# a-rtemis99/hpc_suffix_array

Hardware: AMD Instinct MI355X
Metric: suffixes sorted/sec + ms/doubling-round, 1 GiB input at 1/2/4/8 MI355X (higher is better)
Workload: dtype u32

## Files before the change

hpc_suffix_array_amd/_native.py:

```python
from __future__ import annotations

import ctypes
import os
import subprocess

PKG_DIR = os.path.dirname(os.path.abspath(__file__))
LIB_PATH = os.path.join(PKG_DIR, "lib", "libsa_hip.so")
LIB_PATH = os.environ.get("SA_LIB_PATH", LIB_PATH)
CSRC = os.path.join(PKG_DIR, "csrc")

SA_MAX_ROUNDS = 64
KERNEL_KINDS = ["init", "hist_first", "hist_keys", "scan", "scatter_first", "scatter_keys",
                "heads", "heads_scan", "rerank", "seg_count", "seg_scan", "seg_write", "alphabet", "pack",
                "sort_u", "windows", "local_sort", "pivot_keys", "pivot_count", "pivot_write"]
SCHEDULE_PACKED = 0
SCHEDULE_REFERENCE = 1
ROUND1_AUTO = 0
ROUND1_LSD = 1
ROUND1_BUCKETED = 2
SA_K_COUNT = len(KERNEL_KINDS)
FIND_AUTO = 0
FIND_LANE = 1
FIND_WAVE = 2
FIND_LANE_MAX = 3584
# ... 101 lines not shown
            "round_ms": list(self.round_ms[:r]),
            "distinct": [int(x) for x in self.distinct[:r]],
            "passes": list(self.passes[:r]),
            "sorted_n": [int(x) for x in self.sorted_n[:r]],
            "prefix_len": [int(x) for x in self.prefix_len[:r]],
            "schedule": "reference" if self.schedule == SCHEDULE_REFERENCE else "packed",
            "init_chars": self.init_chars,
            "sigma": self.sigma,
            "sparse_ranks": bool(self.sparse_ranks),
            "round1": {ROUND1_LSD: "lsd", ROUND1_BUCKETED: "bucketed", 3: "pivot"}.get(self.round1, "lsd"),
            "largest_window": self.largest_window,
            "round1_segments": {0: "exact", 1: "padded", 2: "padded-overflow", 3: "striped-records",
                                4: "striped-records-overflow"}.get(self.round1_segments, "exact"),
            "round1_layout": {"compact": bool(self.round1_layout & 1), "pk8": bool(self.round1_layout & 2),
                              "xq": bool(self.round1_layout & 4), "eonly": bool(self.round1_layout & 8)},
            "reference_model_bytes": int(self.model_bytes),
            "round_bytes": [int(x) for x in self.round_bytes[:r]],
            "round1_windows": [int(x) for x in self.round1_windows],
            "alphabet": {0: "exact", 1: "sampled", 2: "refuted"}.get(self.alphabet, "exact"),
            "kernels": {k: {"ms": self.kern_ms[i], "launches": int(self.kern_launches[i]),
                            "bytes": int(self.kern_bytes[i])} for i, k in enumerate(KERNEL_KINDS)},
        }


DIST_OK = 0
DIST_UNSUPPORTED = 1
DIST_UNBALANCED = 2


class SaDistInfo(ctypes.Structure):
# ... 182 lines not shown
```

hpc_suffix_array_amd/csrc/sa_build.hip:

```cpp
#include <hip/hip_runtime.h>

#include <algorithm>
#include <atomic>
#include <chrono>
#include <cstdarg>
#include <cstdio>
#include <cstdlib>
#include <cstring>
#include <mutex>
#include <string>
#include <thread>
#include <vector>

#include "../../include/sa_hip.h"

#ifndef SA_ALPHA_GRID
#define SA_ALPHA_GRID 2048
#endif

#include "sa_bucket.h"
#include "sa_check.h"
#include "sa_kernels.h"
#include "sa_lcp.h"
#include "sa_limits.h"
// ... 122 lines not shown
    uint32_t* counts = nullptr;
    uint32_t* words = nullptr;
    uint32_t* alpha = nullptr;
    uint16_t* code = nullptr;
    uint32_t* host_words = nullptr;
    hipEvent_t ev[sa::kEvPool + sa::kRoundEv + 1];
    int ev_ready = 0;
    sa::DistState* dist = nullptr;
    uint32_t dbg = 0;
    int32_t span_extra = 0;
    int32_t tune = 0;
    bool dna = false;
    bool alpha_prove = false;
    bool alpha_refuted = false;
    bool samples_pending = false;
};

namespace sa {

static uint64_t pad_capacity(uint64_t n) { return n + n / 8 + (1ull << 22); }

static uint64_t pad_elems(uint64_t n) {
    const uint64_t m = align_up(std::max<uint64_t>(n, 1), 64);
    return (n >= (1ull << 26) && n <= (1ull << 31)) ? align_up(pad_capacity(n), 64) : m;
}

constexpr uint64_t kMaxRadix = 1024;
static uint64_t tile_states_bytes(uint64_t n) { return ((n + kTile - 1) / kTile + 1) * kMaxRadix * 8; }

static uint64_t ws_bytes(uint64_t n) {
// ... 1091 lines not shown
        if (sampled) {
            const bool first4k = (c->dbg & SA_DEBUG_ALPHA_SAMPLE_SMALL) != 0;
            const uint64_t nb = alpha_text_blocks(n), ns = alpha_sample_blocks(n, first4k);
            hipLaunchKernelGGL(k_alphabet_sample, dim3((uint32_t)std::min<uint64_t>(ns, 2ull * (uint32_t)c->cus)),
                               dim3(kBlock), 0, s, d_text, n, nb, ns, c->alpha);
            add_bytes(st, SA_K_ALPHABET, alpha_sample_bytes(n, first4k));
        } else {
            const uint32_t grid = (uint32_t)std::min<uint64_t>((n + kBlock * 16 - 1) / (kBlock * 16), SA_ALPHA_GRID);
            hipLaunchKernelGGL(k_alphabet, dim3(grid), dim3(kBlock), 0, s, d_text, n, c->alpha);
            add_bytes(st, SA_K_ALPHABET, n);
        }
        tm.end();
        SA_HIP(hipGetLastError());
        SA_HIP(hipMemcpyAsync(h_alpha, c->alpha, 8 * 4, hipMemcpyDeviceToHost, s));
        SA_HIP(hipMemcpyAsync(h_tail, d_text + (n - tail_n), tail_n, hipMemcpyDeviceToHost, s));
        SA_HIP(host_sync(s));
        *complete = true;
        for (uint32_t t = 0; t < tail_n; ++t) {
            const uint32_t x = h_tail[t];
            if (!((h_alpha[x >> 5] >> (x & 31)) & 1u)) *complete = false;
            h_alpha[x >> 5] |= 1u << (x & 31);
        }
        sigma = 0;
        for (int b = 0; b < 256; ++b) h_code[b] = ((h_alpha[b >> 5] >> (b & 31)) & 1u) ? (uint16_t)(++sigma) : 0;
        SA_HIP(hipMemcpyAsync(c->code, h_code, 256 * 2, hipMemcpyHostToDevice, s));
        c->dna = sigma == 4 && h_code['A'] && h_code['C'] && h_code['G'] && h_code['T'];
        K = choose_chars(sigma, n, opts ? opts->init_chars : 0);
        Kb = (opts && opts->init_chars > 0) || sigma <= 1 ? K : min_chars(sigma, n);
        bucketed = plan_bucketed(sigma, n, Kb, r1, c->radix, &bp, 1, (c->dbg & SA_DEBUG_NO_CMP) ? 0 : 1);
        if (bucketed && bp.bs.cmp && short_suffix_ties(h_tail, n, tail_n, h_code, sigma, bp.bs.s, bp.bs.R))
            bucketed = plan_bucketed(sigma, n, Kb, r1, c->radix, &bp, 1, 0);
// ... 19 lines not shown
    bool r1_pivot = false;
    uint64_t D = 0, m = 0, G = 0;
    uint64_t seg1[3] = {0, 0, 0};
    int r2 = 0;
    for (;;) {
        bool complete = true;
        rc = plan_round1(sampled, &complete);
        if (rc) return rc;
        if (sampled && !(bucketed && complete)) {
            SA_TRACE("packed: sampled alphabet (sigma=%u) not kept: %s", sigma,
                     complete ? "round 1 is not bucketed" : "the tail holds another symbol");
            sampled = false;
            continue;
        }
        c->samples_pending = false;
        if (!bucketed) break;
        bool done = false;
        c->alpha_prove = sampled && sigma < 256;
        c->alpha_refuted = false;
        rc = round1_bucketed(c, d_text, n, d_sa, bp, full_range(bp, n), s, tm, st, &done, &fused, seg1, &ksh1, true,
                             true, &r2);
        c->alpha_prove = false;
        if (rc) return rc;
        if (c->alpha_refuted) {
            SA_TRACE("packed: the first pass met a symbol outside the sampled alphabet, again with the exact one");
            sampled = false;
            refuted = true;
            continue;
        }
        bucketed = done;
        if (done) {
            keys1 = c->keys[0];
            P = 2;
            K = bp.K;
        }
        break;
    }
// ... 209 lines not shown
    if (st) st->schedule = schedule;
    if (n == 0) return SA_OK;
    if (!d_text || !d_sa) return set_err(SA_E_INVALID, "NULL device pointer");
    if (n > 0xFFFFFFFFull) return set_err(SA_E_INVALID, "n = %llu exceeds 2^32-1 on one device",
                                          (unsigned long long)n);
    if (schedule != SA_SCHEDULE_PACKED && schedule != SA_SCHEDULE_REFERENCE)
        return set_err(SA_E_INVALID, "unknown schedule %d", schedule);
    SA_HIP(hipSetDevice(c->device));
    int rc = ensure_capacity(c, n);
    if (rc) return rc;
    Timer tm{c, s, opts && opts->profile, st};
    c->radix = opts ? opts->radix : 0;
    set_debug(c, opts);
    if (c->radix != 0 && c->radix != 1) return set_err(SA_E_INVALID, "unknown radix algorithm %d", c->radix);
    SA_HIP(hipMemsetAsync(c->words, 0, 64, s));
    Events ev;
    rc = ev.make();
    if (rc) return rc;
    SA_TRACE("build n=%llu schedule=%d", (unsigned long long)n, schedule);
    SA_HIP(hipEventRecord(ev.e[0], s));
    if (n == 1) {
        SA_HIP(hipMemsetAsync(d_sa, 0, 4, s));
    } else if (schedule == SA_SCHEDULE_REFERENCE) {
        rc = build_reference(c, d_text, n, d_sa, s, st, tm);
    } else {
        rc = build_packed(c, d_text, n, d_sa, s, opts, st, tm);
    }
    if (rc) return rc;
    SA_HIP(hipEventRecord(ev.e[1], s));
    SA_HIP(hipEventSynchronize(ev.e[1]));
// ... 805 lines not shown
```

hpc_suffix_array_amd/csrc/sa_dist.h:

```cpp
#pragma once
#ifndef SA_COARSE_WPC
#define SA_COARSE_WPC 4
#endif


constexpr int kDistMaxWorld = 1024;

struct DistState {
    uint64_t n = 0;
    int world = 1, rank = 0;
    uint32_t sigma = 0, K = 0;
    bool planned = false;
    const uint8_t* text = nullptr;
    BucketPlan bp;
    std::vector<uint32_t> cut;
    uint32_t blo = 0, bhi = 0;
    uint64_t m = 0, sa_off = 0, mcap = 0;
    uint32_t* sa = nullptr;
    uint32_t ksh = 0;
    uint64_t cap_n = 0, cap_m = 0;
    uint16_t* owner_tab = nullptr;
    uint32_t* gmember = nullptr;
    uint32_t* gprefix = nullptr;
    uint32_t* crank = nullptr;
// ... 405 lines not shown
        info->groups = 0;
        return SA_OK;
    }
    BucketRange br;
    br.blo = d->blo;
    br.bhi = d->bhi;
    br.m = d->m;
    br.sa_off = d->sa_off;
    br.always_u = true;
    br.rank = d->crank;
    br.member = d->gmember;
    br.prefix = d->gprefix;
    br.tmp_rank = d->perm;
    bool done = false, fused = false;
    uint64_t seg[3] = {0, 0, 0};
    int rc = round1_bucketed(c, d_text, d->n, d_sa, d->bp, br, s, tm, st, &done, &fused, seg, &d->ksh);
    d->sa = d_sa;
    tm.flush();
    if (rc) return rc;
    if (!done || !fused) {
        info->round1_ok = 0;
        return SA_OK;
    }
    d->mu = seg[1];
    d->gu = seg[2];
    d->uo = 0;
    d->rounds = 1;
    info->heads = seg[0];
    info->unsorted = seg[1];
    info->groups = seg[2];
// ... 151 lines not shown
```

hpc_suffix_array_amd/csrc/sa_round1.h:

```cpp
#pragma once

#ifndef SA_HIST_WPC
#define SA_HIST_WPC 64
#endif
#ifndef SA_REC_STRIPED
#define SA_REC_STRIPED 1
#endif
#ifndef SA_BB_EXTRA
#define SA_BB_EXTRA 0
#endif
#ifndef SA_ITEMS_A
#define SA_ITEMS_A 12
#endif
#ifndef SA_TEXT_BLOCK
#define SA_TEXT_BLOCK 512
#endif
#ifndef SA_LIST_BLOCK
#define SA_LIST_BLOCK 1024
#endif


#ifndef SA_SEG_BLOCK
#define SA_SEG_BLOCK 1024
#endif
// ... 154 lines not shown
};

static BucketRange full_range(const BucketPlan& bp, uint64_t n) {
    BucketRange r;
    r.blo = 0;
    r.bhi = 1u << bp.bs.bb;
    r.m = n;
    return r;
}

static uint32_t range_hb(uint32_t nb) {
    const uint32_t w = bit_width(nb > 1 ? nb - 1 : 1);
    return std::max<uint32_t>(7u, w > kLoBits ? w - kLoBits : 0u);
}

static int round1_bucketed(sa_context* c, const uint8_t* d_text, uint64_t n, uint32_t* d_sa, const BucketPlan& bp,
                           const BucketRange& br_, hipStream_t s, Timer& tm, sa_stats* st, bool* done, bool* fused,
                           uint64_t seg[3], uint32_t* ksh, bool allow_pad = true, bool allow_xq = true,
                           int* round2 = nullptr) {
    *done = false;
    *fused = false;
    *ksh = 0;
    if (round2) *round2 = 0;
    const uint64_t m = br_.m;
    const uint32_t blo = br_.blo, bhi = br_.bhi;
    if (bhi <= blo || bhi - blo > (1u << 18)) return set_err(SA_E_INTERNAL, "bucket range [%u, %u)", blo, bhi);
    int rc = onesweep_prepare(c, s);
    if (rc) return rc;
    SA_HIP(hipMemsetAsync(c->words, 0, 12, s));
    SA_HIP(hipMemsetAsync(c->words + 5, 0, 28, s));
    const bool listed = m * 10 <= n * 3;
    uint64_t* const lkeys = c->keys_u;
    uint32_t* const lpos = c->vals_u;
    const uint64_t rtiles = (n + kTile - 1) / kTile;
    const uint32_t rgrid = (uint32_t)(std::min<uint64_t>(rtiles, (uint64_t)SA_HIST_WPC * (uint32_t)c->cus) /
                                      kRecStripes * kRecStripes);
    const uint64_t rcap64 = (c->dbg & SA_DEBUG_PAD_OVERFLOW) ? m / kRecStripes / 2 + 1
                                                             : (m + m / 8) / kRecStripes + 2 * (uint64_t)kTile;
    const bool striped = SA_REC_STRIPED && listed && allow_pad && !(c->dbg & SA_DEBUG_NO_PAD) &&
                         rtiles >= 4ull * kRecStripes && rgrid >= kRecStripes && kRecStripes * rcap64 <= c->ucap;
    const uint32_t rcap = (uint32_t)std::min<uint64_t>(rcap64, UINT32_MAX);
    uint32_t* const rcur = c->hist;
    const bool padded = allow_pad && !listed && blo == 0 && bhi == (1u << bp.bs.bb) && n >= kPadMinN &&
                        n <= kPadMaxN && c->cap_pad >= pad_capacity(n) && !(c->dbg & SA_DEBUG_NO_PAD);
    const uint32_t ssh = std::max<uint32_t>(6u, bit_width(n) > 21 ? bit_width(n) - 21 : 0u);
// ... 73 lines not shown
    const bool np2 = (bp.bs.sigma & (bp.bs.sigma - 1)) != 0;
    const bool pk8 = plan_pk8(bp, hb, c->dbg, !br_.always_u);
    uint32_t bits1 = 0;
    if (bp.bs.cmp) {
        const uint64_t ps = bp.bs.pow_s1 * bp.bs.sigma, per = (ps + (1ull << bp.bs.bb) - 1) >> bp.bs.bb;
        const bool exact = (ps & ((1ull << bp.bs.bb) - 1)) == 0;
        bits1 = bit_width(exact ? per - 1 : per) + bp.bs.rb;
        if (c->span_extra > 0) bits1 = std::min<uint32_t>(bits1 + (uint32_t)c->span_extra, 64u - bp.ib);
    }
    const bool fast32 = bits1 > (uint32_t)kSubBits && bits1 - kSubBits <= kLowMax &&
                        (m / (uint64_t)(bhi - blo) >= 4ull * kWinStride || (c->dbg & SA_DEBUG_FAST32_SMALL)) &&
                        !(c->dbg & SA_DEBUG_NO_FAST32);
    static_assert(kXqQueues == kXq && kXqRegionSlack == kXqSlack, "sa_limits.h mirrors sa_split.h");
    const bool xq = SA_SEG_XQ && allow_xq && fast32 && c->cus % (int)kXq == 0 && !(c->dbg & SA_DEBUG_NO_XQ) &&
                    c->kucap >= xq_region_space(m) + kWave && xq_offsets_fit(m);
    if (st) st->round1_layout = (bp.bs.cmp ? 1 : 0) | (pk8 ? 2 : 0) | (xq ? 4 : 0) | (bp.bs.cmp == 2 ? 8 : 0);
    const uint64_t xqw = xq_words(1u << hb);
    uint32_t* xq_dh = nullptr;
    uint32_t* xq_pc = nullptr;
    uint32_t* xq_pn = nullptr;
    if (xq) {
        const uint64_t need = xqw + 1032 + 2ull * kXq * nb_tab;
        if (c->segx_words < need) {
            hipFree(c->segx);
            c->segx = nullptr;
            c->segx_words = 0;
            if (hipMalloc(&c->segx, need * 4) != hipSuccess) {
                (void)hipGetLastError();
                return set_err(SA_E_NOMEM, "second-pass queue workspace (%llu words)", (unsigned long long)need);
            }
            c->segx_words = need;
        }
        xq_dh = c->segx + xqw;
        xq_pc = xq_dh + 1032;
        xq_pn = xq_pc + (uint64_t)kXq * nb_tab;
    }
    uint32_t* const g_lo = os_ghist(c);
    uint32_t* const g_hi = os_ghist(c) + kLoRadix;
    const uint32_t stripes = padded ? text_stripes(c) : 1u;
    uint32_t* const cursor = stripes > 1 ? c->hist : os_ghist(c) + 5 * kRadix;
    uint32_t* const cursor_sum = stripes > 1 ? c->hist + kMaxStripes * kLoRadix : cursor;
    if (stripes > 1) SA_HIP(hipMemsetAsync(cursor, 0, (size_t)stripes * kLoRadix * 4, s));
    if (!padded) {
        tm.begin(SA_K_SCAN);
        hipLaunchKernelGGL(k_digit_base_wide, dim3(1), dim3(1024), 0, s, (const uint32_t*)g_lo, kLoRadix, os_base(c));
        tm.end();
    }
    tm.begin(SA_K_SCATTER_FIRST);
    {
        constexpr int kItemsA = SA_ITEMS_A;
        constexpr int kTextBlock = SA_TEXT_BLOCK;
        const bool pow2 = (bp.bs.sigma & (bp.bs.sigma - 1)) == 0;
        const bool dna = SA_DNA_SWAR && c->dna && bp.bs.s + bp.bs.R + kItemsA - 1 <= 32 && 2 * bp.bs.s <= 32;
        const bool ident = SA_TEXT_IDENT && bp.bs.sigma == 256 && bp.bs.s + bp.bs.R <= 8 && bp.bs.s <= 4;
        uint32_t* const alpha_bad = c->alpha_prove && !listed ? c->words + kAlphaBadWord : nullptr;
        auto text_grid = [&](int block) {
            const uint64_t tile = (uint64_t)block * kItemsA;
            return (uint32_t)std::max<uint64_t>(
                1, std::min<uint64_t>((n + tile - 1) / tile, (uint64_t)c->cus * (kSpBlock / block)));
        };
#define SA_TEXT_PASS(P, PK, BLK, DNA, ID)                                                                     \
    hipLaunchKernelGGL((k_split_text<kItemsA, BLK, P, PK, DNA, ID>), dim3(text_grid(BLK)), dim3(BLK), 0, s, d_text, n, \
                       (const uint16_t*)c->code, bp.bs, (const uint32_t*)(padded ? pstart : os_base(c)),           \
                       os_tickets(c), c->keys[0], c->vals_alt, g_hi, cursor, m, blo, bhi,                          \
                       padded ? (const uint32_t*)pstart + 1 : nullptr, padded ? c->words + 11 : nullptr, hb, bp.ib, \
                       stripes, alpha_bad)
        if (listed) {
            constexpr int kItemsL = SA_ITEMS_B, kListBlock = SA_LIST_BLOCK;
            const uint64_t tl = (uint64_t)kListBlock * kItemsL;
            const uint32_t gl = (uint32_t)std::max<uint64_t>(
                1, std::min<uint64_t>((m + tl - 1) / tl, (uint64_t)c->cus * (kSpBlock / kListBlock)));
            if (pk8)
                hipLaunchKernelGGL((k_split_list<kItemsL, kListBlock, true>), dim3(gl), dim3(kListBlock), 0, s, bp.bs,
                                   (const uint64_t*)lkeys, (const uint32_t*)lpos, m, blo, (const uint32_t*)os_base(c),
                                   os_tickets(c), c->keys[0], c->vals_alt, g_hi, cursor, hb, bp.ib,
                                   striped ? (const uint32_t*)rcur : nullptr, rcap);
            else
                hipLaunchKernelGGL((k_split_list<kItemsL, kListBlock, false>), dim3(gl), dim3(kListBlock), 0, s, bp.bs,
                                   (const uint64_t*)lkeys, (const uint32_t*)lpos, m, blo, (const uint32_t*)os_base(c),
                                   os_tickets(c), c->keys[0], c->vals_alt, g_hi, cursor, 0u, 0u,
                                   striped ? (const uint32_t*)rcur : nullptr, rcap);
        } else if (pk8 && np2) {
#define SA_TEXT_NP2(R32)                                                                                         \
    hipLaunchKernelGGL((k_split_text<kItemsA, kSpBlock, false, true, false, false, R32>), dim3(text_grid(kSpBlock)), \
                       dim3(kSpBlock), 0, s, d_text, n, (const uint16_t*)c->code, bp.bs,                           \
                       (const uint32_t*)(padded ? pstart : os_base(c)), os_tickets(c), c->keys[0], c->vals_alt, g_hi, \
                       cursor, m, blo, bhi, padded ? (const uint32_t*)pstart + 1 : nullptr,                        \
                       padded ? c->words + 11 : nullptr, hb, bp.ib, stripes, alpha_bad)
            if (bp.bs.powR1 * (uint64_t)bp.bs.sigma <= 0xFFFFFFFFull && !(((uint32_t)c->tune >> 28) & 1u))
                SA_TEXT_NP2(true);
            else
                SA_TEXT_NP2(false);
#undef SA_TEXT_NP2
        } else if (pk8 && dna) {
            SA_TEXT_PASS(true, true, kTextBlock, true, false);
        } else if (pk8 && ident) {
            SA_TEXT_PASS(true, true, kTextBlock, false, true);
        } else if (pk8) {
            SA_TEXT_PASS(true, true, kTextBlock, false, false);
        } else if (pow2 && ident) {
            SA_TEXT_PASS(true, false, kTextBlock, false, true);
        } else if (pow2) {
            SA_TEXT_PASS(true, false, kTextBlock, false, false);
        } else if (bp.bs.powR1 * (uint64_t)bp.bs.sigma <= 0xFFFFFFFFull && !(((uint32_t)c->tune >> 28) & 1u)) {
            hipLaunchKernelGGL((k_split_text<kItemsA, kSpBlock, false, false, false, false, true>),
                               dim3(text_grid(kSpBlock)), dim3(kSpBlock), 0, s, d_text, n, (const uint16_t*)c->code,
                               bp.bs, (const uint32_t*)(padded ? pstart : os_base(c)), os_tickets(c), c->keys[0],
                               c->vals_alt, g_hi, cursor, m, blo, bhi, padded ? (const uint32_t*)pstart + 1 : nullptr,
                               padded ? c->words + 11 : nullptr, hb, bp.ib, stripes, alpha_bad);
        } else {
            SA_TEXT_PASS(false, false, kSpBlock, false, false);
        }
#undef SA_TEXT_PASS
    }
    tm.end();
    add_bytes(st, SA_K_SCATTER_FIRST, listed ? (pk8 ? 20 : 24) * m : n + (pk8 ? 8 : 12) * m);
    tm.begin(SA_K_SCAN);
    hipLaunchKernelGGL(k_digit_base_wide, dim3(1), dim3(1024), 0, s, (const uint32_t*)g_hi, 1u << hb,
                       os_base(c) + kLoRadix);
    if (xq)
        hipLaunchKernelGGL(k_xq_dh, dim3(1), dim3(1024), 0, s, (const uint32_t*)g_hi, 1u << hb,
                           (c->dbg & SA_DEBUG_XQ_OVERFLOW) ? 1u : 0u, xq_dh);
    if (padded) {
        if (stripes > 1)
            hipLaunchKernelGGL(k_sum_rows, dim3(1), dim3(kLoRadix), 0, s, (const uint32_t*)cursor, stripes, cursor_sum);
        hipLaunchKernelGGL(k_digit_base_wide, dim3(1), dim3(1024), 0, s, (const uint32_t*)cursor_sum, kLoRadix, dlo);
    }
    tm.end();
    tm.begin(SA_K_SCATTER_KEYS);
    {
        constexpr int kItemsB = SA_ITEMS_B, kItemsPk = SA_ITEMS_PK;
        const SrcBucketKeys sb{c->keys[0], c->vals_alt, bp.bs.rb, bp.bs.bsh, bp.bs.cmul, blo};
        const SrcPk8 sp{c->keys[0]};
        uint32_t* tk = os_tickets(c) + 1;
        const uint32_t* hbase = os_base(c) + kLoRadix;
        SA_HIP(hipMemsetAsync(c->segw, 0, segw_words(1u << hb) * 4, s));
        SegXq sx;
        if (xq) {
            SA_HIP(hipMemsetAsync(c->segx, 0, xqw * 4, s));
            sx.cur = c->segx;
            sx.sbase = reinterpret_cast<uint64_t*>(c->segx + (uint64_t)kXq * kSegs * (1u << hb));
            sx.done = c->segx + 3ull * kXq * kSegs * (1u << hb);
            sx.tickets = sx.done + kXq * kSegs;
            sx.dh = xq_dh;
            sx.err2 = c->words + 9;
            sx.cap = (uint32_t)std::min<uint64_t>(c->kucap, UINT32_MAX);
        }
        constexpr int kSegBlock = SA_SEG_BLOCK;
        const int sblk = hb <= 9 ? kSegBlock : kSpBlock;
        const uint64_t ut = (uint64_t)sblk * (pk8 ? kItemsPk : kItemsB);
        const uint64_t units = (m + ut - 1) / ut + kSegs;
        const uint32_t grid = xq ? (uint32_t)c->cus * (kSpBlock / sblk)
                                 : (uint32_t)std::max<uint64_t>(1, std::min<uint64_t>(units, (uint64_t)c->cus * (kSpBlock / sblk)));
        switch (hb) {
// ... 274 lines not shown
```

hpc_suffix_array_amd/csrc/sa_split.h:

```cpp
#pragma once
#include <type_traits>
#include "sa_alpha.h"
#include "sa_bucket.h"
#include "sa_onesweep.h"

#ifndef SA_SEG_PROF
#define SA_SEG_PROF 0
#endif
#ifndef SA_TEXT_PROF
#define SA_TEXT_PROF 0
#endif

namespace sa {

constexpr int kSpBlock = 1024;
constexpr int kSpItems = 8;
constexpr int kSpTile = kSpBlock * kSpItems;
constexpr int kSpWaves = kSpBlock / kWave;

__device__ __forceinline__ uint32_t wave_min_u32(uint32_t x) {
#pragma unroll
    for (int o = kWave / 2; o > 0; o >>= 1) x = min(x, (uint32_t)__shfl_xor((int)x, o, kWave));
    return x;
}
// ... 227 lines not shown
#ifndef SA_TEXT_LOAD16
#define SA_TEXT_LOAD16 1
#endif
#ifndef SA_TEXT_SCAN1
#define SA_TEXT_SCAN1 1
#endif
#ifndef SA_TEXT_TAB1
#define SA_TEXT_TAB1 1
#endif
#ifndef SA_TEXT_EARLY
#define SA_TEXT_EARLY 1
#endif
#ifndef SA_TEXT_TPT
#define SA_TEXT_TPT 4
#endif
template <int ITEMS, int BLOCK = kSpBlock, bool POW2 = false, bool PK8 = false, bool DNA = false, bool IDENT = false,
          bool R32 = false>
__global__ __launch_bounds__(BLOCK, 2048 / BLOCK) void k_split_text(const uint8_t* __restrict__ text, uint64_t n,
                                                         const uint16_t* __restrict__ code, BucketSpec b,
                                                         const uint32_t* __restrict__ digit_base,
                                                         uint32_t* __restrict__ ticket, uint64_t* __restrict__ out_keys,
                                                         uint32_t* __restrict__ out_vals,
                                                         uint32_t* __restrict__ ghist_hi, uint32_t* __restrict__ cursor,
                                                         uint64_t m, uint32_t blo, uint32_t bhi,
                                                         const uint32_t* __restrict__ seg_end = nullptr,
                                                         uint32_t* __restrict__ ovf = nullptr, uint32_t pk_hb = 0,
                                                         uint32_t pk_ib = 0, uint32_t stripes = 1,
                                                         uint32_t* __restrict__ alpha_bad = nullptr) {
    constexpr bool NP2 = PK8 && !POW2;
    constexpr int RADIX = kLoRadix;
    constexpr int RWAVES = RADIX / kWave;
    constexpr int TILE = BLOCK * ITEMS;
    constexpr int kHalo = kMaxK;
    constexpr int NW = (TILE + kHalo) / 4;
    constexpr int WPT = (NW + BLOCK - 1) / BLOCK;
    static_assert(ITEMS % 4 == 0 && kHalo % 4 == 0 && TILE <= 65535, "word staging, 16-bit tile offsets");
    constexpr bool LD16 = SA_TEXT_LOAD16 != 0, SCAN1 = SA_TEXT_SCAN1 != 0, TAB1 = SA_TEXT_TAB1 != 0;
    constexpr bool EARLY = SA_TEXT_EARLY != 0;
    constexpr int NC = NW / 4;
    static_assert(!LD16 || (NW % 4 == 0 && NC <= BLOCK && WPT <= 4), "one 16-byte chunk per lane");
    static_assert(!SCAN1 || RADIX == 4 * kWave, "wave 0 scans four digits per lane");
    __shared__ uint64_t s_keys[TILE];
    __shared__ uint16_t s_idx[TILE];
    __shared__ __attribute__((aligned(16))) uint32_t s_dcw[(DNA && LD16) ? 4 : NW + 8];
    __shared__ uint32_t s_pkw[DNA ? (NW + 3) / 4 + 4 : 1];
    __shared__ uint8_t s_map[256];
    __shared__ __attribute__((aligned(16))) uint32_t s_cnt[RADIX];
    __shared__ __attribute__((aligned(8))) uint16_t s_start[RADIX];
    constexpr uint32_t kTabSkip = ~0u;
    __shared__ uint32_t s_gofs[RADIX];
    __shared__ uint32_t s_tmp[RWAVES];
    __shared__ uint32_t s_tile[2];
    __shared__ uint32_t s_kept;
    __shared__ uint32_t s_hhi[1024];
    __shared__ uint32_t s_gend[RADIX];
    const uint8_t* s_dc = reinterpret_cast<const uint8_t*>(s_dcw);
    const uint32_t bspan = bhi - blo;
    bool over = false;
// ... 309 lines not shown
#pragma unroll
        for (int j = 0; j < ITEMS; ++j) {
            const uint32_t d = dr[j] >> 16;
            if (d < (uint32_t)RADIX) {
                const uint32_t pos = s_start[d] + (dr[j] & 0xFFFFu);
                if constexpr (NP2) {
                    const uint32_t cm32 = (uint32_t)b.cmul;
                    const uint64_t prod = (uint64_t)(uint32_t)(k[j] >> b.rb) * cm32;
                    const uint32_t bk = (uint32_t)(prod >> b.bsh);
                    const uint32_t f = (uint32_t)(prod & fmask);
                    uint32_t rd = (uint32_t)((double)f * icm);
                    rd = ((uint64_t)rd * cm32 > f) ? rd - 1u : rd;
                    rd = ((uint64_t)(rd + 1u) * cm32 <= f) ? rd + 1u : rd;
                    const uint32_t hi = (bk - blo) >> kLoBits;
                    const uint64_t rel = ((uint64_t)rd << b.rb) | (k[j] & ((1ull << b.rb) - 1ull));
                    s_keys[pos] = ((uint64_t)hi << (64u - pk_hb)) | (rel << pk_ib) | (tb + ITEMS * dg + j);
                    s_idx[pos] = (uint16_t)d;
                } else if constexpr (PK8) {
                    const uint32_t hi = ((uint32_t)(k[j] >> kbsh) - blo) >> kLoBits;
                    s_keys[pos] = ((uint64_t)hi << (64u - pk_hb)) | ((k[j] & remmask) << pk_ib) |
                                  (tb + ITEMS * dg + j);
                    s_idx[pos] = (uint16_t)d;
                } else {
                    s_keys[pos] = k[j];
                    s_idx[pos] = (uint16_t)(ITEMS * dg + j);
                }
            }
        }
        if constexpr (TAB1) {
            if (dg < (uint32_t)RADIX) {
                uint32_t dgo = dg;
                asm volatile("" : "+v"(dgo));
                const uint64_t g0 = (uint64_t)dbase + clm;
                const uint64_t gend = seg_end ? (uint64_t)s_gend[dgo] : m;
                const uint32_t gw = (uint32_t)g0 - s_start[dgo];
                const bool fits = g0 + tile_cnt <= gend && gw != kTabSkip;
                if (tile_cnt && !fits) over = true;
// ... 4 lines not shown
        }
        __syncthreads();
        TEXT_STAMP(3)
        if constexpr (EARLY) {
            uint32_t tk;
            if (dg == 0) tk = next_tile();
            if (tn < tiles) stage(tn);
            if (dg == 0) s_tile[par] = tk;
            TEXT_STAMP(0)
        }
        const uint32_t kept = s_kept;
#pragma unroll
        for (int j = 0; j < ITEMS; ++j) {
            const uint32_t q = j * BLOCK + dg;
            if (q < kept) {
                const uint64_t key = s_keys[q];
                uint32_t dd;
                if constexpr (PK8) {
                    dd = s_idx[q];
                } else {
                    const uint32_t bq = POW2 ? (uint32_t)(key >> (b.rb + (uint32_t)__builtin_ctz(b.sigma) * b.s - b.bb))
                                             : (uint32_t)(((key >> b.rb) * b.cmul) >> b.bsh);
                    dd = (bq - blo) & (RADIX - 1);
                }
                if constexpr (TAB1) {
                    const uint32_t gw = s_gofs[dd];
                    if (gw != kTabSkip) {
                        const uint32_t g = gw + q;
                        out_keys[g] = key;
                        if constexpr (!PK8) out_vals[g] = (uint32_t)(tb + s_idx[q]);
                    }
                } else {
                    const uint64_t g = (uint64_t)s_gofs[dd] + (q - s_start[dd]);
// ... 197 lines not shown
constexpr uint64_t kBstartWords = (1ull << 18) + 1;

constexpr uint32_t kXqSlack = 2048;
constexpr uint32_t kXqTicketStride = 32;
struct SegXq {
    uint32_t* cur = nullptr;
    uint64_t* sbase = nullptr;
    uint32_t* done = nullptr;
    uint32_t* tickets = nullptr;
    const uint32_t* dh = nullptr;
    uint32_t cap = 0;
    uint32_t* err2 = nullptr;
};
constexpr uint64_t xq_words(int radix) { return 3ull * kXq * kSegs * radix + kXq * kSegs + kXq * kXqTicketStride; }

template <class Src, int RBITS, int ITEMS, int BLOCK = kSpBlock, bool XQ = false>
__global__ __launch_bounds__(BLOCK, 2048 / BLOCK) void k_split_seg(Src src, uint64_t n, uint32_t shift,
                                                        const uint32_t* __restrict__ lo_base,
                                                        const uint32_t* __restrict__ digit_base,
                                                        uint32_t* __restrict__ segw, uint32_t* __restrict__ ticket,
                                                        uint32_t ib, uint64_t* __restrict__ out_w,
                                                        uint32_t* __restrict__ err,
                                                        const uint32_t* __restrict__ seg_cnt = nullptr,
                                                        const uint32_t* __restrict__ dense_lo = nullptr,
                                                        uint32_t stripes = 1, SegXq xq = SegXq{}) {
    constexpr int RADIX = 1 << RBITS;
    constexpr int RWAVES = RADIX / kWave;
    constexpr int WTILE = kWave * ITEMS;
    constexpr int TILE = BLOCK * ITEMS;
    static_assert(BLOCK >= RADIX && (int)kSegs <= BLOCK, "one thread per digit / segment");
    static_assert((int)(kSegs * kMaxStripes) <= 2 * BLOCK, "two sub-segments per thread in the unit numbering");
    static_assert(TILE <= 65535, "16-bit tile offsets");
    __shared__ uint64_t s_keys[TILE];
    __shared__ uint16_t s_dig[TILE];
    __shared__ uint32_t s_dmin[RADIX];
    __shared__ uint32_t s_cnt[RADIX];
    __shared__ uint16_t s_start[RADIX];
    __shared__ uint32_t s_gofs[RADIX];
    __shared__ uint32_t s_tmp[(BLOCK / kWave)];
    __shared__ uint32_t s_ubase[kSegs * kMaxStripes + 1];
    __shared__ uint32_t s_tile[2];
    __shared__ uint32_t s_last;
    __shared__ uint32_t s_claim[RADIX];
    const uint32_t xqq = XQ ? (blockIdx.x & (kXq - 1)) : 0u;
    uint32_t* const cur = XQ ? xq.cur + (uint64_t)xqq * kSegs * RADIX : segw;
    uint64_t* const sbase = XQ ? xq.sbase + (uint64_t)xqq * kSegs * RADIX
                               : reinterpret_cast<uint64_t*>(segw + (uint64_t)kSegs * RADIX);
    uint32_t* const done = XQ ? xq.done + xqq * kSegs : segw + 3ull * kSegs * RADIX;
    if constexpr (XQ) ticket = xq.tickets + xqq * kXqTicketStride;
// ... 116 lines not shown
            if (XQ ? qcount(s_ubase[l * stripes]) == 0 : dlo[l] == 0) {
                bh = XQ ? xqq * xrs + xq.dh[dg] : digit_base[dg];
            } else {
                uint64_t w;
                uint32_t spins = 0;
                while (((w = __hip_atomic_load(&sbase[(uint64_t)l * RADIX + dg], __ATOMIC_RELAXED,
                                               __HIP_MEMORY_SCOPE_AGENT)) & kReady) == 0) {
                    if (++spins > kSpinLimit) {
                        atomicOr(err, 1u);
                        break;
                    }
                    __builtin_amdgcn_s_sleep(1);
                }
                bh = (uint32_t)w;
            }
            s_gofs[dg] = bh + s_claim[dg];
            if constexpr (XQ) {
                if (tile_cnt && (uint64_t)bh + s_claim[dg] + tile_cnt > (uint64_t)xqq * xrs + xq.dh[dg + 1])
                    atomicOr(xq.err2, 1u);
            }
            s_claim[dg] = bh;
            if constexpr (!Src::kPk8) s_dmin[dg] = bucket_dmin(((dg << kLoBits) | l) + src.bofs, src.cmul, src.bsh);
        }
        __syncthreads();
        SEG_STAMP(2)
        if (s_last) {
            if (dg < (uint32_t)RADIX) {
                const uint32_t tot = __hip_atomic_load(&cur[(uint64_t)l * RADIX + dg], __ATOMIC_RELAXED,
                                                       __HIP_MEMORY_SCOPE_AGENT);
                for (uint32_t l2 = l + 1; l2 < kSegs; ++l2) {
                    __hip_atomic_store(&sbase[(uint64_t)l2 * RADIX + dg], kReady | (uint64_t)(s_claim[dg] + tot),
                                       __ATOMIC_RELAXED, __HIP_MEMORY_SCOPE_AGENT);
                    if (units_of(l2) > 0) break;
                }
// ... 1 lines not shown
        }
        __syncthreads();
        const uint32_t un = unit_of((uint32_t)__builtin_amdgcn_readfirstlane((int)s_tile[par ^ 1u]));
        SEG_STAMP(3)
        uint32_t ln = l, validn = valid;
        uint64_t tbn = tb;
        if (un < units) locate(un, ln, tbn, validn);
        uint64_t kn[ITEMS];
        uint32_t vn[ITEMS];
        load(tbn, validn, kn, vn);
#pragma unroll
        for (int j = 0; j < ITEMS; ++j) {
            const uint32_t d = dr[j] >> 16;
            if (d < (uint32_t)RADIX) {
                const uint32_t pos = s_start[d] + (dr[j] & 0xFFFFu);
                if constexpr (Src::kPk8)
                    s_keys[pos] = k[j] & ((1ull << shift) - 1ull);
                else
                    s_keys[pos] = ((k[j] - ((uint64_t)s_dmin[d] << src.rb)) << ib) | v[j];
                s_dig[pos] = (uint16_t)d;
            }
        }
        __syncthreads();
        SEG_STAMP(4)
        if (dg < (uint32_t)RADIX) s_cnt[dg] = 0;
#pragma unroll
        for (int j = 0; j < ITEMS; ++j) {
            const uint32_t q = j * BLOCK + dg;
            if (q < valid) {
                const uint32_t dd = s_dig[q];
                const uint64_t g = (uint64_t)s_gofs[dd] + (q - s_start[dd]);
                if (g < gcap) out_w[g] = s_keys[q];
            }
        }
        __syncthreads();
        SEG_STAMP(5)
#pragma unroll
        for (int j = 0; j < ITEMS; ++j) {
            k[j] = kn[j];
            v[j] = vn[j];
        }
        u = un;
        l = ln;
        tb = tbn;
        valid = validn;
        par ^= 1u;
    }
// ... 84 lines not shown
```

Measured before the change: 110.7 billion.

## Carry scatter digit inside packed first-pass items and preclear round-1 state early

In the first text split pass, the 8-bit digit and tile-local offset are now packed into the low bits of each 64-bit item, so the separate shared-memory s_idx array is no longer needed. The item is rebuilt with the tile base when it is written out. Round-1 buffer clears (onesweep prepare, words, hist, segw, segx) are issued while the host waits on the alphabet readback, so they overlap the host sync instead of following it. Segment-pass variants (item digit, single offset table) are added behind macros that are off by default. This saves LDS and shared-memory traffic, at the cost of needing ib to hold the offset and digit bits, plus extra state flags that must be reset on every path.

```diff
diff --git a/hpc_suffix_array_amd/_native.py b/hpc_suffix_array_amd/_native.py
--- a/hpc_suffix_array_amd/_native.py
+++ b/hpc_suffix_array_amd/_native.py
@@ -139,6 +139,7 @@
                                 4: "striped-records-overflow"}.get(self.round1_segments, "exact"),
             "round1_layout": {"compact": bool(self.round1_layout & 1), "pk8": bool(self.round1_layout & 2),
                               "xq": bool(self.round1_layout & 4), "eonly": bool(self.round1_layout & 8)},
+            "first_pass_item_digit": bool(self.round1_layout & 16),
             "reference_model_bytes": int(self.model_bytes),
             "round_bytes": [int(x) for x in self.round_bytes[:r]],
             "round1_windows": [int(x) for x in self.round1_windows],
diff --git a/hpc_suffix_array_amd/csrc/sa_build.hip b/hpc_suffix_array_amd/csrc/sa_build.hip
--- a/hpc_suffix_array_amd/csrc/sa_build.hip
+++ b/hpc_suffix_array_amd/csrc/sa_build.hip
@@ -160,6 +160,8 @@
     bool alpha_prove = false;
     bool alpha_refuted = false;
     bool samples_pending = false;
+    bool r1_clean = false;
+    uint64_t r1_clean_segx = 0;
 };
 
 namespace sa {
@@ -1281,7 +1283,14 @@
         SA_HIP(hipGetLastError());
         SA_HIP(hipMemcpyAsync(h_alpha, c->alpha, 8 * 4, hipMemcpyDeviceToHost, s));
         SA_HIP(hipMemcpyAsync(h_tail, d_text + (n - tail_n), tail_n, hipMemcpyDeviceToHost, s));
-        SA_HIP(host_sync(s));
+        if (c->radix == 0 && r1 != SA_ROUND1_LSD) {
+            SA_HIP(hipEventRecord(c->ev[kSyncEv], s));
+            const int prc = round1_preclear(c, s);
+            if (prc) return prc;
+            SA_HIP(host_sync_event(c->ev[kSyncEv]));
+        } else {
+            SA_HIP(host_sync(s));
+        }
         *complete = true;
         for (uint32_t t = 0; t < tail_n; ++t) {
             const uint32_t x = h_tail[t];
@@ -1331,13 +1340,17 @@
             continue;
         }
         c->samples_pending = false;
-        if (!bucketed) break;
+        if (!bucketed) {
+            c->r1_clean = false;
+            break;
+        }
         bool done = false;
         c->alpha_prove = sampled && sigma < 256;
         c->alpha_refuted = false;
         rc = round1_bucketed(c, d_text, n, d_sa, bp, full_range(bp, n), s, tm, st, &done, &fused, seg1, &ksh1, true,
                              true, &r2);
         c->alpha_prove = false;
+        c->r1_clean = false;
         if (rc) return rc;
         if (c->alpha_refuted) {
             SA_TRACE("packed: the first pass met a symbol outside the sampled alphabet, again with the exact one");
@@ -1577,6 +1590,7 @@
     set_debug(c, opts);
     if (c->radix != 0 && c->radix != 1) return set_err(SA_E_INVALID, "unknown radix algorithm %d", c->radix);
     SA_HIP(hipMemsetAsync(c->words, 0, 64, s));
+    c->r1_clean = false;
     Events ev;
     rc = ev.make();
     if (rc) return rc;
diff --git a/hpc_suffix_array_amd/csrc/sa_dist.h b/hpc_suffix_array_amd/csrc/sa_dist.h
--- a/hpc_suffix_array_amd/csrc/sa_dist.h
+++ b/hpc_suffix_array_amd/csrc/sa_dist.h
@@ -443,6 +443,7 @@
     br.tmp_rank = d->perm;
     bool done = false, fused = false;
     uint64_t seg[3] = {0, 0, 0};
+    c->r1_clean = false;
     int rc = round1_bucketed(c, d_text, d->n, d_sa, d->bp, br, s, tm, st, &done, &fused, seg, &d->ksh);
     d->sa = d_sa;
     tm.flush();
diff --git a/hpc_suffix_array_amd/csrc/sa_itemdig.h b/hpc_suffix_array_amd/csrc/sa_itemdig.h
--- /dev/null
+++ b/hpc_suffix_array_amd/csrc/sa_itemdig.h
@@ -0,0 +1,40 @@
+#pragma once
+#include <stdint.h>
+
+#if defined(__HIPCC__) || defined(__HIP__)
+#define SA_IDG_HD __host__ __device__ __forceinline__
+#else
+#define SA_IDG_HD inline
+#endif
+
+namespace sa {
+
+constexpr uint32_t kIdgDigitBits = 8;
+
+constexpr uint32_t idg_offset_bits(uint32_t tile) {
+    uint32_t b = 0;
+    for (uint32_t x = tile - 1; x; x >>= 1) ++b;
+    return b;
+}
+
+constexpr bool idg_fits(uint32_t ib, uint32_t ob) { return ib <= 32 && ib >= ob + kIdgDigitBits; }
+
+SA_IDG_HD uint64_t pk8_item(uint32_t hi, uint64_t rel, uint64_t pos, uint32_t hb, uint32_t ib) {
+    return ((uint64_t)hi << (64u - hb)) | (rel << ib) | pos;
+}
+
+SA_IDG_HD uint64_t idg_pack(uint32_t hi, uint64_t rel, uint32_t d, uint32_t off, uint32_t hb, uint32_t ib,
+                            uint32_t ob) {
+    return pk8_item(hi, rel, (d << ob) | off, hb, ib);
+}
+
+SA_IDG_HD uint32_t idg_digit(uint32_t lo, uint32_t ob) { return (lo >> ob) & ((1u << kIdgDigitBits) - 1u); }
+SA_IDG_HD uint32_t idg_offset(uint32_t lo, uint32_t ob) { return lo & ((1u << ob) - 1u); }
+
+SA_IDG_HD uint64_t idg_rebuild(uint64_t item, uint32_t tb, uint32_t ob) {
+    const uint32_t lo = (uint32_t)item;
+    const uint32_t nlo = (lo & ~(((1u << kIdgDigitBits) - 1u) << ob)) + tb;
+    return (item & 0xFFFFFFFF00000000ull) | nlo;
+}
+
+}
diff --git a/hpc_suffix_array_amd/csrc/sa_round1.h b/hpc_suffix_array_amd/csrc/sa_round1.h
--- a/hpc_suffix_array_amd/csrc/sa_round1.h
+++ b/hpc_suffix_array_amd/csrc/sa_round1.h
@@ -192,6 +192,21 @@
     return std::max<uint32_t>(7u, w > kLoBits ? w - kLoBits : 0u);
 }
 
+static int round1_preclear(sa_context* c, hipStream_t s) {
+    int rc = onesweep_prepare(c, s);
+    if (rc) return rc;
+    SA_HIP(hipMemsetAsync(c->words, 0, 48, s));
+    SA_HIP(hipMemsetAsync(c->hist, 0, (size_t)kMaxStripes * kLoRadix * 4, s));
+    SA_HIP(hipMemsetAsync(c->segw, 0, segw_words(1024) * 4, s));
+    c->r1_clean_segx = 0;
+    if (c->segx) {
+        c->r1_clean_segx = std::min<uint64_t>(c->segx_words, xq_words(1024));
+        SA_HIP(hipMemsetAsync(c->segx, 0, c->r1_clean_segx * 4, s));
+    }
+    c->r1_clean = true;
+    return SA_OK;
+}
+
 static int round1_bucketed(sa_context* c, const uint8_t* d_text, uint64_t n, uint32_t* d_sa, const BucketPlan& bp,
                            const BucketRange& br_, hipStream_t s, Timer& tm, sa_stats* st, bool* done, bool* fused,
                            uint64_t seg[3], uint32_t* ksh, bool allow_pad = true, bool allow_xq = true,
@@ -203,10 +218,14 @@
     const uint64_t m = br_.m;
     const uint32_t blo = br_.blo, bhi = br_.bhi;
     if (bhi <= blo || bhi - blo > (1u << 18)) return set_err(SA_E_INTERNAL, "bucket range [%u, %u)", blo, bhi);
-    int rc = onesweep_prepare(c, s);
-    if (rc) return rc;
-    SA_HIP(hipMemsetAsync(c->words, 0, 12, s));
-    SA_HIP(hipMemsetAsync(c->words + 5, 0, 28, s));
+    const bool clean = c->r1_clean;
+    c->r1_clean = false;
+    if (!clean) {
+        int rc = onesweep_prepare(c, s);
+        if (rc) return rc;
+        SA_HIP(hipMemsetAsync(c->words, 0, 12, s));
+        SA_HIP(hipMemsetAsync(c->words + 5, 0, 28, s));
+    }
     const bool listed = m * 10 <= n * 3;
     uint64_t* const lkeys = c->keys_u;
     uint32_t* const lpos = c->vals_u;
@@ -310,14 +329,20 @@
     static_assert(kXqQueues == kXq && kXqRegionSlack == kXqSlack, "sa_limits.h mirrors sa_split.h");
     const bool xq = SA_SEG_XQ && allow_xq && fast32 && c->cus % (int)kXq == 0 && !(c->dbg & SA_DEBUG_NO_XQ) &&
                     c->kucap >= xq_region_space(m) + kWave && xq_offsets_fit(m);
-    if (st) st->round1_layout = (bp.bs.cmp ? 1 : 0) | (pk8 ? 2 : 0) | (xq ? 4 : 0) | (bp.bs.cmp == 2 ? 8 : 0);
+    const bool np2_r32 = np2 && bp.bs.powR1 * (uint64_t)bp.bs.sigma <= 0xFFFFFFFFull && !(((uint32_t)c->tune >> 28) & 1u);
+    const bool idg = SA_TEXT_ITEMDIG && pk8 && !listed && !np2_r32 &&
+                     idg_fits(bp.ib, idg_offset_bits((np2 ? kSpBlock : SA_TEXT_BLOCK) * SA_ITEMS_A));
+    if (st)
+        st->round1_layout = (bp.bs.cmp ? 1 : 0) | (pk8 ? 2 : 0) | (xq ? 4 : 0) | (bp.bs.cmp == 2 ? 8 : 0) | (idg ? 16 : 0);
     const uint64_t xqw = xq_words(1u << hb);
     uint32_t* xq_dh = nullptr;
     uint32_t* xq_pc = nullptr;
     uint32_t* xq_pn = nullptr;
+    bool segx_fresh = false;
     if (xq) {
         const uint64_t need = xqw + 1032 + 2ull * kXq * nb_tab;
         if (c->segx_words < need) {
+            segx_fresh = true;
             hipFree(c->segx);
             c->segx = nullptr;
             c->segx_words = 0;
@@ -336,7 +361,10 @@
     const uint32_t stripes = padded ? text_stripes(c) : 1u;
     uint32_t* const cursor = stripes > 1 ? c->hist : os_ghist(c) + 5 * kRadix;
     uint32_t* const cursor_sum = stripes > 1 ? c->hist + kMaxStripes * kLoRadix : cursor;
-    if (stripes > 1) SA_HIP(hipMemsetAsync(cursor, 0, (size_t)stripes * kLoRadix * 4, s));
+    static_assert(kBstartOff >= segw_words(1024), "round1_preclear clears c->segw below the bucket tables");
+    if (stripes > 1 && !clean) SA_HIP(hipMemsetAsync(cursor, 0, (size_t)stripes * kLoRadix * 4, s));
+    if (!clean) SA_HIP(hipMemsetAsync(c->segw, 0, segw_words(1u << hb) * 4, s));
+    if (xq && !(clean && !segx_fresh && c->r1_clean_segx >= xqw)) SA_HIP(hipMemsetAsync(c->segx, 0, xqw * 4, s));
     if (!padded) {
         tm.begin(SA_K_SCAN);
         hipLaunchKernelGGL(k_digit_base_wide, dim3(1), dim3(1024), 0, s, (const uint32_t*)g_lo, kLoRadix, os_base(c));
@@ -355,8 +383,10 @@
             return (uint32_t)std::max<uint64_t>(
                 1, std::min<uint64_t>((n + tile - 1) / tile, (uint64_t)c->cus * (kSpBlock / block)));
         };
-#define SA_TEXT_PASS(P, PK, BLK, DNA, ID)                                                                     \
-    hipLaunchKernelGGL((k_split_text<kItemsA, BLK, P, PK, DNA, ID>), dim3(text_grid(BLK)), dim3(BLK), 0, s, d_text, n, \
+#define SA_TEXT_PASS(P, PK, BLK, DNA, ID) SA_TEXT_PASS_G(P, PK, BLK, DNA, ID, false)
+#define SA_TEXT_PASS_G(P, PK, BLK, DNA, ID, IDG)                                                              \
+    hipLaunchKernelGGL((k_split_text<kItemsA, BLK, P, PK, DNA, ID, false, IDG>), dim3(text_grid(BLK)), dim3(BLK), 0, s, \
+                       d_text, n,                                                                              \
                        (const uint16_t*)c->code, bp.bs, (const uint32_t*)(padded ? pstart : os_base(c)),           \
                        os_tickets(c), c->keys[0], c->vals_alt, g_hi, cursor, m, blo, bhi,                          \
                        padded ? (const uint32_t*)pstart + 1 : nullptr, padded ? c->words + 11 : nullptr, hb, bp.ib, \
@@ -377,23 +407,25 @@
                                    os_tickets(c), c->keys[0], c->vals_alt, g_hi, cursor, 0u, 0u,
                                    striped ? (const uint32_t*)rcur : nullptr, rcap);
         } else if (pk8 && np2) {
-#define SA_TEXT_NP2(R32)                                                                                         \
-    hipLaunchKernelGGL((k_split_text<kItemsA, kSpBlock, false, true, false, false, R32>), dim3(text_grid(kSpBlock)), \
+#define SA_TEXT_NP2_G(R32, IDG)                                                                                  \
+    hipLaunchKernelGGL((k_split_text<kItemsA, kSpBlock, false, true, false, false, R32, IDG>), dim3(text_grid(kSpBlock)), \
                        dim3(kSpBlock), 0, s, d_text, n, (const uint16_t*)c->code, bp.bs,                           \
                        (const uint32_t*)(padded ? pstart : os_base(c)), os_tickets(c), c->keys[0], c->vals_alt, g_hi, \
                        cursor, m, blo, bhi, padded ? (const uint32_t*)pstart + 1 : nullptr,                        \
                        padded ? c->words + 11 : nullptr, hb, bp.ib, stripes, alpha_bad)
-            if (bp.bs.powR1 * (uint64_t)bp.bs.sigma <= 0xFFFFFFFFull && !(((uint32_t)c->tune >> 28) & 1u))
-                SA_TEXT_NP2(true);
-            else
-                SA_TEXT_NP2(false);
-#undef SA_TEXT_NP2
+            if (np2_r32) SA_TEXT_NP2_G(true, false);
+            else if (idg) SA_TEXT_NP2_G(false, true);
+            else SA_TEXT_NP2_G(false, false);
+#undef SA_TEXT_NP2_G
         } else if (pk8 && dna) {
-            SA_TEXT_PASS(true, true, kTextBlock, true, false);
+            if (idg) SA_TEXT_PASS_G(true, true, kTextBlock, true, false, true);
+            else SA_TEXT_PASS(true, true, kTextBlock, true, false);
         } else if (pk8 && ident) {
-            SA_TEXT_PASS(true, true, kTextBlock, false, true);
+            if (idg) SA_TEXT_PASS_G(true, true, kTextBlock, false, true, true);
+            else SA_TEXT_PASS(true, true, kTextBlock, false, true);
         } else if (pk8) {
-            SA_TEXT_PASS(true, true, kTextBlock, false, false);
+            if (idg) SA_TEXT_PASS_G(true, true, kTextBlock, false, false, true);
+            else SA_TEXT_PASS(true, true, kTextBlock, false, false);
         } else if (pow2 && ident) {
             SA_TEXT_PASS(true, false, kTextBlock, false, true);
         } else if (pow2) {
@@ -408,6 +440,7 @@
             SA_TEXT_PASS(false, false, kSpBlock, false, false);
         }
 #undef SA_TEXT_PASS
+#undef SA_TEXT_PASS_G
     }
     tm.end();
     add_bytes(st, SA_K_SCATTER_FIRST, listed ? (pk8 ? 20 : 24) * m : n + (pk8 ? 8 : 12) * m);
@@ -430,10 +463,8 @@
         const SrcPk8 sp{c->keys[0]};
         uint32_t* tk = os_tickets(c) + 1;
         const uint32_t* hbase = os_base(c) + kLoRadix;
-        SA_HIP(hipMemsetAsync(c->segw, 0, segw_words(1u << hb) * 4, s));
         SegXq sx;
         if (xq) {
-            SA_HIP(hipMemsetAsync(c->segx, 0, xqw * 4, s));
             sx.cur = c->segx;
             sx.sbase = reinterpret_cast<uint64_t*>(c->segx + (uint64_t)kXq * kSegs * (1u << hb));
             sx.done = c->segx + 3ull * kXq * kSegs * (1u << hb);
diff --git a/hpc_suffix_array_amd/csrc/sa_split.h b/hpc_suffix_array_amd/csrc/sa_split.h
--- a/hpc_suffix_array_amd/csrc/sa_split.h
+++ b/hpc_suffix_array_amd/csrc/sa_split.h
@@ -1,6 +1,7 @@
 #pragma once
 #include <type_traits>
 #include "sa_alpha.h"
+#include "sa_itemdig.h"
 #include "sa_bucket.h"
 #include "sa_onesweep.h"
 
@@ -265,8 +266,11 @@
 #ifndef SA_TEXT_TPT
 #define SA_TEXT_TPT 4
 #endif
+#ifndef SA_TEXT_ITEMDIG
+#define SA_TEXT_ITEMDIG 1
+#endif
 template <int ITEMS, int BLOCK = kSpBlock, bool POW2 = false, bool PK8 = false, bool DNA = false, bool IDENT = false,
-          bool R32 = false>
+          bool R32 = false, bool IDG = false>
 __global__ __launch_bounds__(BLOCK, 2048 / BLOCK) void k_split_text(const uint8_t* __restrict__ text, uint64_t n,
                                                          const uint16_t* __restrict__ code, BucketSpec b,
                                                          const uint32_t* __restrict__ digit_base,
@@ -289,10 +293,12 @@
     constexpr bool LD16 = SA_TEXT_LOAD16 != 0, SCAN1 = SA_TEXT_SCAN1 != 0, TAB1 = SA_TEXT_TAB1 != 0;
     constexpr bool EARLY = SA_TEXT_EARLY != 0;
     constexpr int NC = NW / 4;
+    constexpr uint32_t OB = idg_offset_bits(TILE);
+    static_assert(!IDG || (PK8 && kLoBits == (int)kIdgDigitBits), "the digit rides in packed items only");
     static_assert(!LD16 || (NW % 4 == 0 && NC <= BLOCK && WPT <= 4), "one 16-byte chunk per lane");
     static_assert(!SCAN1 || RADIX == 4 * kWave, "wave 0 scans four digits per lane");
     __shared__ uint64_t s_keys[TILE];
-    __shared__ uint16_t s_idx[TILE];
+    __shared__ uint16_t s_idx[IDG ? 1 : TILE];
     __shared__ __attribute__((aligned(16))) uint32_t s_dcw[(DNA && LD16) ? 4 : NW + 8];
     __shared__ uint32_t s_pkw[DNA ? (NW + 3) / 4 + 4 : 1];
     __shared__ uint8_t s_map[256];
@@ -632,13 +638,21 @@
                     rd = ((uint64_t)(rd + 1u) * cm32 <= f) ? rd + 1u : rd;
                     const uint32_t hi = (bk - blo) >> kLoBits;
                     const uint64_t rel = ((uint64_t)rd << b.rb) | (k[j] & ((1ull << b.rb) - 1ull));
-                    s_keys[pos] = ((uint64_t)hi << (64u - pk_hb)) | (rel << pk_ib) | (tb + ITEMS * dg + j);
-                    s_idx[pos] = (uint16_t)d;
+                    if constexpr (IDG) {
+                        s_keys[pos] = idg_pack(hi, rel, d, ITEMS * dg + j, pk_hb, pk_ib, OB);
+                    } else {
+                        s_keys[pos] = ((uint64_t)hi << (64u - pk_hb)) | (rel << pk_ib) | (tb + ITEMS * dg + j);
+                        s_idx[pos] = (uint16_t)d;
+                    }
                 } else if constexpr (PK8) {
                     const uint32_t hi = ((uint32_t)(k[j] >> kbsh) - blo) >> kLoBits;
-                    s_keys[pos] = ((uint64_t)hi << (64u - pk_hb)) | ((k[j] & remmask) << pk_ib) |
-                                  (tb + ITEMS * dg + j);
-                    s_idx[pos] = (uint16_t)d;
+                    if constexpr (IDG) {
+                        s_keys[pos] = idg_pack(hi, k[j] & remmask, d, ITEMS * dg + j, pk_hb, pk_ib, OB);
+                    } else {
+                        s_keys[pos] = ((uint64_t)hi << (64u - pk_hb)) | ((k[j] & remmask) << pk_ib) |
+                                      (tb + ITEMS * dg + j);
+                        s_idx[pos] = (uint16_t)d;
+                    }
                 } else {
                     s_keys[pos] = k[j];
                     s_idx[pos] = (uint16_t)(ITEMS * dg + j);
@@ -673,9 +687,12 @@
         for (int j = 0; j < ITEMS; ++j) {
             const uint32_t q = j * BLOCK + dg;
             if (q < kept) {
-                const uint64_t key = s_keys[q];
+                uint64_t key = s_keys[q];
                 uint32_t dd;
-                if constexpr (PK8) {
+                if constexpr (IDG) {
+                    dd = idg_digit((uint32_t)key, OB);
+                    key = idg_rebuild(key, (uint32_t)tb, OB);
+                } else if constexpr (PK8) {
                     dd = s_idx[q];
                 } else {
                     const uint32_t bq = POW2 ? (uint32_t)(key >> (b.rb + (uint32_t)__builtin_ctz(b.sigma) * b.s - b.bb))
@@ -903,6 +920,12 @@
 };
 constexpr uint64_t xq_words(int radix) { return 3ull * kXq * kSegs * radix + kXq * kSegs + kXq * kXqTicketStride; }
 
+#ifndef SA_SEG_ITEMDIG
+#define SA_SEG_ITEMDIG 0
+#endif
+#ifndef SA_SEG_TAB1
+#define SA_SEG_TAB1 0
+#endif
 template <class Src, int RBITS, int ITEMS, int BLOCK = kSpBlock, bool XQ = false>
 __global__ __launch_bounds__(BLOCK, 2048 / BLOCK) void k_split_seg(Src src, uint64_t n, uint32_t shift,
                                                         const uint32_t* __restrict__ lo_base,
@@ -920,8 +943,10 @@
     static_assert(BLOCK >= RADIX && (int)kSegs <= BLOCK, "one thread per digit / segment");
     static_assert((int)(kSegs * kMaxStripes) <= 2 * BLOCK, "two sub-segments per thread in the unit numbering");
     static_assert(TILE <= 65535, "16-bit tile offsets");
+    constexpr bool IDIG = SA_SEG_ITEMDIG != 0 && Src::kPk8, TAB1 = SA_SEG_TAB1 != 0;
+    constexpr uint32_t kTabSkip = ~0u;
     __shared__ uint64_t s_keys[TILE];
-    __shared__ uint16_t s_dig[TILE];
+    __shared__ uint16_t s_dig[IDIG ? 1 : TILE];
     __shared__ uint32_t s_dmin[RADIX];
     __shared__ uint32_t s_cnt[RADIX];
     __shared__ uint16_t s_start[RADIX];
@@ -1068,10 +1093,22 @@
                 }
                 bh = (uint32_t)w;
             }
-            s_gofs[dg] = bh + s_claim[dg];
-            if constexpr (XQ) {
-                if (tile_cnt && (uint64_t)bh + s_claim[dg] + tile_cnt > (uint64_t)xqq * xrs + xq.dh[dg + 1])
-                    atomicOr(xq.err2, 1u);
+            if constexpr (TAB1) {
+                const uint64_t g0 = (uint64_t)bh + s_claim[dg];
+                const uint32_t gw = (uint32_t)g0 - s_start[dg];
+                bool fits = g0 + tile_cnt <= gcap;
+                if constexpr (XQ) {
+                    const bool in = g0 + tile_cnt <= (uint64_t)xqq * xrs + xq.dh[dg + 1] && gw != kTabSkip;
+                    if (tile_cnt && !in) atomicOr(xq.err2, 1u);
+                    fits = fits && in;
+                }
+                s_gofs[dg] = fits ? gw : kTabSkip;
+            } else {
+                s_gofs[dg] = bh + s_claim[dg];
+                if constexpr (XQ) {
+                    if (tile_cnt && (uint64_t)bh + s_claim[dg] + tile_cnt > (uint64_t)xqq * xrs + xq.dh[dg + 1])
+                        atomicOr(xq.err2, 1u);
+                }
             }
             s_claim[dg] = bh;
             if constexpr (!Src::kPk8) s_dmin[dg] = bucket_dmin(((dg << kLoBits) | l) + src.bofs, src.cmul, src.bsh);
@@ -1103,11 +1140,13 @@
             const uint32_t d = dr[j] >> 16;
             if (d < (uint32_t)RADIX) {
                 const uint32_t pos = s_start[d] + (dr[j] & 0xFFFFu);
-                if constexpr (Src::kPk8)
+                if constexpr (IDIG)
+                    s_keys[pos] = k[j];
+                else if constexpr (Src::kPk8)
                     s_keys[pos] = k[j] & ((1ull << shift) - 1ull);
                 else
                     s_keys[pos] = ((k[j] - ((uint64_t)s_dmin[d] << src.rb)) << ib) | v[j];
-                s_dig[pos] = (uint16_t)d;
+                if constexpr (!IDIG) s_dig[pos] = (uint16_t)d;
             }
         }
         __syncthreads();
@@ -1117,9 +1156,21 @@
         for (int j = 0; j < ITEMS; ++j) {
             const uint32_t q = j * BLOCK + dg;
             if (q < valid) {
-                const uint32_t dd = s_dig[q];
-                const uint64_t g = (uint64_t)s_gofs[dd] + (q - s_start[dd]);
-                if (g < gcap) out_w[g] = s_keys[q];
+                uint64_t key = s_keys[q];
+                uint32_t dd;
+                if constexpr (IDIG) {
+                    dd = (uint32_t)(key >> shift);
+                    key &= (1ull << shift) - 1ull;
+                } else {
+                    dd = s_dig[q];
+                }
+                if constexpr (TAB1) {
+                    const uint32_t gw = s_gofs[dd];
+                    if (gw != kTabSkip) out_w[gw + q] = key;
+                } else {
+                    const uint64_t g = (uint64_t)s_gofs[dd] + (q - s_start[dd]);
+                    if (g < gcap) out_w[g] = key;
+                }
             }
         }
         __syncthreads();
```

After: 110.4 billion. About the same (-0.2%).
